# bingjeff/trex-gym

Hardware: AMD Instinct MI355X
Metric: env-steps/sec (whole node), trex.urdf 4096 envs per MI355X (higher is better)
Workload: dtype f32

## Files before the change

trex-gym_amd/csrc/trex_step.hip:

```cpp
#include <hip/hip_runtime.h>
#include <stdint.h>

#include <type_traits>

#include "device_model.h"

#define TL TREX_TL
#define MAXD TREX_MAXD
#define MAXCH TREX_MAXCH
#define MAXC TREX_MAXC

#ifndef TREX_STAMPS
#define TREX_STAMPS 0
#endif
#ifndef TREX_PAIR_MAX
#define TREX_PAIR_MAX 4096
#endif
#ifndef TREX_PAIR_LAUNCH
#define TREX_PAIR_LAUNCH (!TREX_STAMPS)
#endif
#ifndef TREX_ABLATE_EXACT_MATH
#define TREX_ABLATE_EXACT_MATH 0
#endif
#ifndef TREX_ABLATE_EXACT_QUAT
// ... 152 lines not shown
  o[1] = s[1] * v[0] + s[3] * v[1] + s[4] * v[2];
  o[2] = s[2] * v[0] + s[4] * v[1] + s[5] * v[2];
}
__device__ __forceinline__ void sym6_mul(const Sym6 &m, const float *v, float *o) {
  float a[3], b[3], c[3], d[3];
  sym3_mul(m.A, v, a);
  matvec3(m.B, v + 3, b);
  c[0] = m.B[0] * v[0] + m.B[3] * v[1] + m.B[6] * v[2];
  c[1] = m.B[1] * v[0] + m.B[4] * v[1] + m.B[7] * v[2];
  c[2] = m.B[2] * v[0] + m.B[5] * v[1] + m.B[8] * v[2];
  sym3_mul(m.C, v + 3, d);
#pragma unroll
  for (int i = 0; i < 3; i++) { o[i] = a[i] + b[i]; o[3 + i] = c[i] + d[i]; }
}
__device__ __forceinline__ void sym6_full(const Sym6 &m, float *f) {
  const int sidx[3][3] = {{0, 1, 2}, {1, 3, 4}, {2, 4, 5}};
#pragma unroll
  for (int r = 0; r < 3; r++)
#pragma unroll
    for (int c = 0; c < 3; c++) {
      f[6 * r + c] = m.A[sidx[r][c]];
      f[6 * r + 3 + c] = m.B[3 * r + c];
      f[6 * (3 + r) + c] = m.B[3 * c + r];
      f[6 * (3 + r) + 3 + c] = m.C[sidx[r][c]];
    }
}
__device__ __forceinline__ void sym6_rank1_sub(Sym6 &m, const float *U, const float *Us) {
  const int ia[6] = {0, 0, 0, 1, 1, 2}, ib[6] = {0, 1, 2, 1, 2, 2};
#pragma unroll
  for (int k = 0; k < 6; k++) {
    m.A[k] = __builtin_fmaf(-U[ia[k]], Us[ib[k]], m.A[k]);
    m.C[k] = __builtin_fmaf(-U[3 + ia[k]], Us[3 + ib[k]], m.C[k]);
  }
#pragma unroll
  for (int r = 0; r < 3; r++)
#pragma unroll
    for (int c = 0; c < 3; c++) m.B[3 * r + c] = __builtin_fmaf(-U[r], Us[3 + c], m.B[3 * r + c]);
}
__device__ __forceinline__ void cross3_acc(const float *a, const float *b, float &o0, float &o1, float &o2) {
  o0 = __builtin_fmaf(a[1], b[2], __builtin_fmaf(-a[2], b[1], o0));
  o1 = __builtin_fmaf(a[2], b[0], __builtin_fmaf(-a[0], b[2], o1));
  o2 = __builtin_fmaf(a[0], b[1], __builtin_fmaf(-a[1], b[0], o2));
}

struct Chol6 { float l[15], il[6]; };
__device__ __forceinline__ constexpr int lidx(int i, int j) { return i * (i - 1) / 2 + j; }
__device__ __forceinline__ float rsqrt_nr(float s) {
#if TREX_ABLATE_EXACT_MATH
  return 1.0f / sqrtf(s);
#endif
  const float r0 = __builtin_amdgcn_rsqf(s);
  const float e = __builtin_fmaf(-s * r0, r0, 1.0f);
  return __builtin_fmaf(0.5f * r0, e, r0);
}
__device__ __forceinline__ void chol6_factor(const float *a, Chol6 &c) {
#pragma unroll
  for (int j = 0; j < 6; j++) {
    float s = a[6 * j + j];
#pragma unroll
    for (int k = 0; k < j; k++) s -= c.l[lidx(j, k)] * c.l[lidx(j, k)];
    c.il[j] = rsqrt_nr(s);
#pragma unroll
    for (int i = j + 1; i < 6; i++) {
      float t = a[6 * i + j];
#pragma unroll
      for (int k = 0; k < j; k++) t -= c.l[lidx(i, k)] * c.l[lidx(j, k)];
      c.l[lidx(i, j)] = t * c.il[j];
    }
  }
}
__device__ __forceinline__ void chol6_solve(const Chol6 &c, const float *r, float *z) {
  float w[6];
#pragma unroll
  for (int i = 0; i < 6; i++) {
    float t = r[i];
#pragma unroll
    for (int k = 0; k < i; k++) t -= c.l[lidx(i, k)] * w[k];
    w[i] = t * c.il[i];
  }
#pragma unroll
  for (int i = 5; i >= 0; i--) {
    float t = w[i];
#pragma unroll
    for (int k = i + 1; k < 6; k++) t -= c.l[lidx(k, i)] * z[k];
    z[i] = t * c.il[i];
  }
}

constexpr int NJMAX = 25;
constexpr int NROW = NJMAX + 3 * MAXC;
static_assert(NROW == 64, "one constraint row per lane");
#define KROW_LANE(k) ((k) < 3 * MAXC - 1 ? NJMAX + 1 + (k) : 0)
constexpr int CLANE0 = NJMAX + 1;
__device__ __forceinline__ int warm_word(int l) {
  if (l >= 1 && l <= MAXC) return 4 * (l - 1);
  if (l == 0 || l >= CLANE0) { const int k = l == 0 ? 3 * MAXC - 1 : l - CLANE0; return 4 * (k / 3) + 1 + k % 3; }
  return -1;
}
constexpr int BREC = 5;
struct WaveLds {
  float4 body[32 * BREC];
  union {
    struct {
      float aba[32][28];
      float rtab[32][9];
    } t;
    float4 desc[64][4];
    float4 cg[160];
  } u;
  float cpt[MAXC][8];
  float st[6][TL];
  float xch[44];
};
enum { ST_Q, ST_QD, ST_TAU, ST_TARGET, ST_NQD, ST_MDG };
static_assert(sizeof(WaveLds) <= 10240, "16 envs per CU need <= 10 KB of LDS each");
constexpr int CG_WORDS = TREX_CM_WORDS;
struct CgLds {
  unsigned long long best[TL];
  float4 ent[TL][2];
  unsigned cm[CG_WORDS];
};
static_assert(sizeof(CgLds) <= sizeof(WaveLds::u), "contact-generation scratch fits the union area");

struct KernelArgs {
  const TrexDeviceModel *model;
  TrexBatchArrays arr;
  int n_envs;
  const float *actions;
  float *obs;
  float *reward;
  uint8_t *done;
  float *done_f;
  int obs_stride, scal_stride;
  float *penalties;
  const uint8_t *reset_mask;
  int32_t *bal;
  float w_distance, w_energy, w_drift;
  float *debug;
  int n_steps;
  long long step_rows;
  int pen_in_rows;
  float *warm;
  const float *ext;
  float *sens;
};
constexpr int SENS_ROWS = 9;

}

#define WSYNC() do { if (PAIR) __builtin_amdgcn_fence(__ATOMIC_ACQ_REL, "wavefront"); else __syncthreads(); } while (0)
template <bool RESET, bool DEBUG, bool MULTI, bool PAIR = false, bool WARM = false, bool EXT = false, bool SENS = false>
__device__ __forceinline__ void trex_step_body(const KernelArgs &args, const int wg_in) {
  static_assert(!PAIR || (!RESET && !DEBUG && !MULTI), "the pair form exists for the product step launch only");
  static_assert(!(WARM && DEBUG), "the diagnostics dump has no warm-start form");
  static_assert(!EXT || (!RESET && !DEBUG), "the external wrench exists for the product step launches only");
  static_assert(!SENS || !DEBUG, "the diagnostics dump has no contact-sensor form");
  __shared__ WaveLds Wpair[PAIR ? 2 : 1];
  __shared__ __attribute__((aligned(16))) unsigned char Gpair[PAIR ? sizeof(CgLds) : 16];
  const int wave = PAIR ? uni((int)threadIdx.x >> 6) : 0;
  int wave_v = PAIR ? (int)threadIdx.x >> 6 : 0;
  if (PAIR) asm volatile("" : "+v"(wave_v));
  WaveLds &W = Wpair[wave_v];
  __shared__ float4 Wrec[WARM ? (PAIR ? 2 : 1) : 1][MAXC];
  float4 *const Wr = Wrec[WARM ? wave_v : 0];
  const int wg = PAIR ? 2 * wg_in + wave : wg_in;
  const int tid = (int)threadIdx.x & 63;
  const TrexDeviceModel *__restrict__ M = args.model;
  int env = wg;
  int bal_phase = 0;
  if (args.bal) {
    const int32_t *B = args.bal;
    bal_phase = uni(B[TREX_BAL_PHASE]);
    const int32_t *cnt = B + TREX_BAL_COUNTS + TREX_BAL_BINS * bal_phase;
    const int k = wg, q = k >> 10, m = min(1024, args.n_envs - (q << 10));
    int r = q == 0 ? k : (q << 10) + (m - 1 - (k & 1023));
    if (PAIR) {
      const int bq = wg_in >> 9, half = args.n_envs >> 1, bm = min(512, half - (bq << 9));
      const int pidx = bq == 0 ? wg_in : (bq << 9) + (bm - 1 - (wg_in & 511));
      r = wave == 0 ? pidx : args.n_envs - 1 - pidx;
    }
    const int lane_ = tid;
    const int mine = lane_ < TREX_BAL_BINS ? cnt[lane_] : 0;
    int b = TREX_BAL_BINS - 1, total = 0;
#pragma unroll
    for (int c = 0; c < TREX_BAL_BINS; c++) total += rl(mine, c);
    for (; b > 0; b--) {
      const int c = rl(mine, b);
      if (r < c) break;
      r -= c;
    }
    if (total == args.n_envs) {
      env = B[TREX_BAL_LISTS + (size_t)(bal_phase * TREX_BAL_BINS + b) * args.n_envs + r];
      if (env < 0 || env >= args.n_envs) env = wg;
    }
  }
  env = uni(env);

  const int nb = M->nb, maxdepth = M->maxdepth;
  const float dt = PAIR ? uni_sgpr(M->prm[TP_DT]) : M->prm[TP_DT];
  const float inv_dt = PAIR ? uni_sgpr(M->inv_dt) : M->inv_dt;
  const float dt_half = PAIR ? uni_sgpr(0.5f * dt) : 0.5f * dt, dt2_quarter = PAIR ? uni_sgpr(0.25f * dt * dt) : 0.25f * dt * dt;
  const int nj = nb - 1;
  auto Mo = [&]() { const TrexDeviceModel *Mi = M; asm volatile("" : "+s"(Mi)); return Mi; };
  auto lane_id = [&]() {
    int l;
    asm volatile("v_mbcnt_lo_u32_b32 %0, -1, 0\n\tv_mbcnt_hi_u32_b32 %0, -1, %0" : "=v"(l));
    return l;
  };

  float pos[3], quat[4], bv[3], bw[3];
  const float mu = args.arr.domain ? uni(args.arr.friction[env]) : (PAIR ? uni_sgpr(M->prm[TP_FRICTION]) : M->prm[TP_FRICTION]);
  bool motors_on;
  int flags_in = 0, steps_in = 0;
  bool do_reset = false;
  bool bad;
  if (RESET) do_reset = args.reset_mask ? (args.reset_mask[env] != 0) : true;
  if (RESET && !do_reset) {
    if (args.obs && tid >= 1 && tid < nb) {
      float *o = args.obs + (size_t)env * args.obs_stride;
      const int slot = M->obs_slot[tid];
      o[slot] = args.arr.q[(size_t)env * TL + tid];
      o[nj + slot] = args.arr.qd[(size_t)env * TL + tid];
    }
    return;
  }
  {
    const bool is_body = tid < nb, is_joint = tid >= 1 && tid < nb;
    float q = 0.f, qd = 0.f, mtau = 0.f, target = 0.f;
    if (RESET && do_reset) {
#pragma unroll
      for (int c = 0; c < 3; c++) { pos[c] = uni(M->base_pos0[c]); bv[c] = 0.f; bw[c] = 0.f; }
#pragma unroll
      for (int c = 0; c < 4; c++) quat[c] = uni(M->base_quat0[c]);
      q = is_body ? M->q_start[tid & (TL - 1)] : 0.f;
      motors_on = false;
    } else {
      const float *b = args.arr.base + (size_t)env * 16;
#pragma unroll
      for (int c = 0; c < 3; c++) { pos[c] = uni(b[c]); bv[c] = uni(b[7 + c]); bw[c] = uni(b[10 + c]); }
#pragma unroll
      for (int c = 0; c < 4; c++) quat[c] = uni(b[3 + c]);
      flags_in = uni(__float_as_int(b[TREX_BASE_FLAGS]));
      if (tid < TL) {
        q = args.arr.q[(size_t)env * TL + tid];
        qd = args.arr.qd[(size_t)env * TL + tid];
      }
      motors_on = RESET ? ((flags_in & TREX_MOTORS_BIT) != 0) : true;
    }
    steps_in = uni(__float_as_int(args.arr.base[(size_t)env * 16 + TREX_BASE_STEPS]));
    bool badl = !(fabsf(q) < 3.0e38f) || !(fabsf(qd) < 3.0e38f);
#pragma unroll
    for (int k = 0; k < 3; k++) badl |= !(fabsf(pos[k]) < 3.0e38f) || !(fabsf(bv[k]) < 3.0e38f) || !(fabsf(bw[k]) < 3.0e38f);
#pragma unroll
    for (int k = 0; k < 4; k++) badl |= !(fabsf(quat[k]) < 3.0e38f);
    bad = __ballot(badl) != 0ull;
    (void)is_joint;
    if (tid < TL) {
      W.st[ST_Q][tid] = q; W.st[ST_QD][tid] = qd; W.st[ST_TAU][tid] = mtau; W.st[ST_TARGET][tid] = target;
      W.st[ST_NQD][tid] = 0.f;
    }
    if (WARM) {
      const int w = warm_word(tid);
      const float v = RESET ? 0.f : args.warm[(size_t)env * TREX_WARM_WORDS + tid];
      if (w >= 0) reinterpret_cast<float *>(Wr)[w] = v;
    }
  }
  WSYNC();
  const int n_sub = RESET ? (do_reset ? 1 : 0) : M->n_substeps;
#ifndef TREX_PRIO_T1
#define TREX_PRIO_T1 1
#define TREX_PRIO_T2 3
#define TREX_PRIO_T3 6
#endif
  const bool aged_launch = args.n_envs <= 4096;
  const int wave_pair = (wg >> 11) & 1;
  auto set_sweep_priority = [&](int contacts) {
    int v = contacts >= TREX_PRIO_T3 ? 3 : (contacts >= TREX_PRIO_T2 ? 2 : (contacts >= TREX_PRIO_T1 ? 1 : 0));
    v += (aged_launch && wave_pair == 1) ? 1 : 0;
    if (v <= 0) __builtin_amdgcn_s_setprio(0);
    else if (v == 1) __builtin_amdgcn_s_setprio(1);
    else if (v == 2) __builtin_amdgcn_s_setprio(2);
    else __builtin_amdgcn_s_setprio(3);
  };
#ifndef TREX_TREE_HEAVY
#define TREX_TREE_HEAVY 12
#endif
  int prio_nc = 0;
  auto set_tree_priority = [&](int substep) {
    if (!PAIR && TREX_TREE_HEAVY > 0 && prio_nc >= TREX_TREE_HEAVY) { __builtin_amdgcn_s_setprio(3); return; }
    if (aged_launch && ((wave_pair + substep) & 1)) __builtin_amdgcn_s_setprio(1); else __builtin_amdgcn_s_setprio(0);
  };
#if TREX_PRIO_MODE == 1
  if (!RESET) { prio_nc = flags_in & 255; set_tree_priority(0); }
#endif

  const float floor_z = PAIR ? uni_sgpr(M->prm[TP_FLOOR_Z]) : M->prm[TP_FLOOR_Z], margin = PAIR ? uni_sgpr(M->prm[TP_CONTACT_MARGIN]) : M->prm[TP_CONTACT_MARGIN];
  const int iters = M->n_iterations;
  int maxc = M->max_contacts;
  if (maxc > MAXC) maxc = MAXC;

  int stat_nc = 0;
  float stat_imp = 0.f;

  auto forward_kinematics = [&](int lt, int psrc, int depth, float *R, float *r, float *dpar, float *Sa) {
    const TrexDeviceModel *Mi = Mo();
    const int bl = lt & (TL - 1);
    float axis[3], jpos[3], jrot[9];
#pragma unroll
    for (int c = 0; c < 3; c++) { axis[c] = Mi->axis[c][bl]; jpos[c] = Mi->jpos[c][bl]; }
#pragma unroll
    for (int c = 0; c < 9; c++) jrot[c] = Mi->jrot[c][bl];
    const float q = W.st[ST_Q][bl];
    float Rl[9];
    {
      float c = cosf(q), s = sinf(q), t = 1.f - c, rq[9];
      rq[0] = t * axis[0] * axis[0] + c;           rq[1] = t * axis[0] * axis[1] - s * axis[2]; rq[2] = t * axis[0] * axis[2] + s * axis[1];
      rq[3] = t * axis[0] * axis[1] + s * axis[2]; rq[4] = t * axis[1] * axis[1] + c;           rq[5] = t * axis[1] * axis[2] - s * axis[0];
      rq[6] = t * axis[0] * axis[2] - s * axis[1]; rq[7] = t * axis[1] * axis[2] + s * axis[0]; rq[8] = t * axis[2] * axis[2] + c;
      matmul3(jrot, rq, Rl);
    }
    quat_to_mat(quat, R);
    r[0] = r[1] = r[2] = 0.f;
    dpar[0] = dpar[1] = dpar[2] = 0.f;
    for (int d = 1; d <= maxdepth; d++) {
      float pR[9], pr[3];
#pragma unroll
      for (int c = 0; c < 9; c++) pR[c] = wshfl(R[c], psrc);
#pragma unroll
      for (int c = 0; c < 3; c++) pr[c] = wshfl(r[c], psrc);
      if (depth == d) {
        float o[3];
        matmul3(pR, Rl, R);
        matvec3(pR, jpos, o);
#pragma unroll
        for (int c = 0; c < 3; c++) { dpar[c] = o[c]; r[c] = pr[c] + o[c]; }
      }
    }
    matvec3(R, axis, Sa);
    if (!(lt >= 1 && lt < nb)) { Sa[0] = Sa[1] = Sa[2] = 0.f; }
  };

#if TREX_STAMPS
  unsigned long long stamp_last = __builtin_amdgcn_s_memtime();
  int stamp_alive = 0, stamp_lamnz = 0;
  if (args.debug && (threadIdx.x & 63) == 0) args.debug[4096 + 11 * args.n_envs + wg] = (float)env;
#endif
  int age = 0;
  bool time_up = false;
  bool env_bad = false;
  float lift = 0.f, drift = 0.f, energy = 0.f;
  auto finish_step = [&]() {
    const int lt = lane_id();
    const int bl = lt & (TL - 1);
    const bool is_body = lt < nb, is_joint = lt >= 1 && lt < nb;
    float head[3];
    {
      const int parent = is_body ? M->parent[bl] : 0;
      const int psrc = parent < 0 ? 0 : parent;
      const int depth = is_body ? M->depth[bl] : -1;
      float R[9], r[3], dpar[3], Sa[3];
      forward_kinematics(lt, psrc, depth, R, r, dpar, Sa);
      const float hp[3] = {M->head_point[0], M->head_point[1], M->head_point[2]};
      float o[3];
      matvec3(R, hp, o);
      const int hb = M->head_body;
#pragma unroll
      for (int k = 0; k < 3; k++) head[k] = rl(pos[k] + r[k] + o[k], hb);
    }
    float q = W.st[ST_Q][bl], qd = W.st[ST_QD][bl], mtau = W.st[ST_TAU][bl];
    if (lt >= TL) { q = 0.f; qd = 0.f; mtau = 0.f; }
    const float power = wsum(is_joint ? fabsf(qd * mtau) : 0.f);
    lift = uni(args.w_distance * (2.5f - head[2]) * (2.5f - head[2]));
    drift = uni(args.w_drift * (head[0] * head[0] + head[1] * head[1]));
    energy = uni(args.w_energy * power);
    bool badl = !(fabsf(q) < 3.0e38f) || !(fabsf(qd) < 3.0e38f);
#pragma unroll
    for (int k = 0; k < 3; k++) badl |= !(fabsf(pos[k]) < 3.0e38f) || !(fabsf(bv[k]) < 3.0e38f) || !(fabsf(bw[k]) < 3.0e38f);
#pragma unroll
    for (int k = 0; k < 4; k++) badl |= !(fabsf(quat[k]) < 3.0e38f);
    if constexpr (EXT) {
      const float *xw = args.ext + (size_t)env * (6 * TL) + bl;
#pragma unroll
      for (int c = 0; c < 6; c++) badl |= is_body && !(fabsf(xw[c * TL]) < 3.0e38f);
    }
    env_bad = bad || (__ballot(badl) != 0ull);
  };
  auto to_start_pose = [&]() {
#pragma unroll
    for (int k = 0; k < 3; k++) { pos[k] = uni(M->base_pos0[k]); bv[k] = 0.f; bw[k] = 0.f; }
#pragma unroll
    for (int k = 0; k < 4; k++) quat[k] = uni(M->base_quat0[k]);
    const int l = lane_id();
    if (l < TL) {
      W.st[ST_Q][l] = l < nb ? Mo()->q_start[l] : 0.f;
      W.st[ST_QD][l] = 0.f; W.st[ST_TAU][l] = 0.f;
    }
    if (WARM && l < MAXC) Wr[l].x = 0.f;
    WSYNC();
  };
  const int n_launch_steps = MULTI ? args.n_steps : 1;
#pragma unroll 1
  for (int ls = 0; ls < n_launch_steps; ls++) {
  if (!RESET) {
    const int l = lane_id();
    if (l < TL) {
      float target = 0.f;
      if (l >= 1 && l < nb) {
        const TrexDeviceModel *Mi = Mo();
        const float a = args.actions[((size_t)(MULTI ? ls : 0) * args.n_envs + env) * nj + Mi->obs_slot[l]];
        target = fminf(fmaxf(a, Mi->lower[l]), Mi->upper[l]);
      }
      W.st[ST_TARGET][l] = target;
    }
    if (MULTI && ls > 0) { motors_on = true; bad = false; env_bad = false; }
  }
  age = 0; time_up = false;
  if (!RESET && args.arr.max_episode_steps > 0) {
    age = steps_in + 1;
    time_up = age >= args.arr.max_episode_steps;
  }
  const int n_total = n_sub + ((!RESET && time_up) ? 1 : 0);
  int n_loop = n_total;
  int nt_pair[2] = {n_total, n_total};
  if (PAIR) {
    if (lane_id() == 0) W.xch[7] = __int_as_float(n_total);
    __syncthreads();
    nt_pair[0] = uni(__float_as_int(Wpair[0].xch[7])); nt_pair[1] = uni(__float_as_int(Wpair[PAIR ? 1 : 0].xch[7]));
    n_loop = max(nt_pair[0], nt_pair[1]);
  }
#pragma unroll 1
  for (int sub = 0; sub < n_loop; sub++) {
    int lt, bl;
    bool is_body, is_joint;
#define RELANE() do { lt = lane_id(); bl = lt & (TL - 1); is_body = lt < nb; is_joint = lt >= 1 && lt < nb; } while (0)
    int psrc, depth;
    float R[9], r[3];
    float Sa[3], dpar[3];
    int nc = 0;
    const bool act = !PAIR || sub < n_total;
    if (act) {
    if (!RESET && sub == n_sub) {
      finish_step();
      to_start_pose();
      motors_on = false;
    }
    RELANE();
    {
      const TrexDeviceModel *Mi = Mo();
      const int parent = is_body ? Mi->parent[bl] : 0;
      psrc = parent < 0 ? 0 : parent;
      depth = is_body ? Mi->depth[bl] : -1;
    }
    {
      float dpar0[3], Sa0[3];
      forward_kinematics(lt, psrc, depth, R, r, dpar0, Sa0);
      if (lt < TL) {
        float4 *rec = &W.body[BREC * lt];
        rec[0] = make_float4(Sa0[0], Sa0[1], Sa0[2], 0.f);
        rec[1] = make_float4(r[0], r[1], r[2], 0.f);
        rec[3] = make_float4(0.f, 0.f, __int_as_float(psrc + 256 * (depth < 0 ? 255 : depth)), 0.f);
        const TrexDeviceModel *Mi = Mo();
        unsigned ch4 = 0u;
#pragma unroll
        for (int k = 0; k < MAXCH; k++) {
          const int c = is_body ? Mi->child[k][bl] : -1;
          ch4 |= (unsigned)(c < 0 ? 255 : c) << (8 * k);
        }
        rec[4] = make_float4(dpar0[0], dpar0[1], dpar0[2], __uint_as_float(ch4));
      }
    }
    if (PAIR) {
      const int l_ = lane_id();
      if (l_ < TL) {
        float *rt = W.u.t.rtab[l_];
#pragma unroll
        for (int c = 0; c < 9; c++) rt[c] = R[c];
      }
      if (l_ == 0) {
#pragma unroll
        for (int c = 0; c < 3; c++) { W.xch[c] = bw[c]; W.xch[3 + c] = bv[c]; }
        W.xch[6] = __int_as_float(env);
        W.xch[36] = pos[2];
      }
    }
    }
    STAMP(0);
    if (PAIR) { __syncthreads(); SUBSTAMP(16); }
    if (!PAIR || wave == 1) {
    for (int e = 0; e < (PAIR ? 2 : 1); e++) {
    if (PAIR && !(sub < nt_pair[e])) continue;
    WaveLds &E = Wpair[PAIR ? e : 0];
    float posz = pos[2];
    if (PAIR) {
      RELANE();
      posz = E.xch[36];
      if (lt < TL) {
#pragma unroll
        for (int c = 0; c < 9; c++) R[c] = E.u.t.rtab[lt][c];
        const float4 q1_ = E.body[BREC * lt + 1];
        r[0] = q1_.x; r[1] = q1_.y; r[2] = q1_.z;
      }
    }

    nc = 0;
    {
      const TrexDeviceModel *Mi = Mo();
      const int hull_v0 = Mi->hull_start[is_body ? lt : nb], hull_v1 = Mi->hull_start[is_body ? lt + 1 : nb];
      CgLds &G = PAIR ? *reinterpret_cast<CgLds *>(Gpair) : *reinterpret_cast<CgLds *>(&W.u);
      const int nchunk = Mi->nchunk;
      const bool is_chunk = lt < nchunk;
      const int cbody = Mi->chunk_body[bl], cv0 = Mi->chunk_v0[bl], cv1 = is_chunk ? Mi->chunk_v1[bl] : 0;
      float Rz[3], zbc;
      {
        const float zb = posz + r[2] - floor_z;
#pragma unroll
        for (int c = 0; c < 3; c++) Rz[c] = wshfl(R[6 + c], cbody);
        zbc = wshfl(zb, cbody);
      }
      bool near = false;
      if (is_chunk) {
        const float cz = Rz[0] * Mi->chunk_c[0][bl] + Rz[1] * Mi->chunk_c[1][bl] + Rz[2] * Mi->chunk_c[2][bl];
        const float reach = fabsf(Rz[0]) * Mi->chunk_h[0][bl] + fabsf(Rz[1]) * Mi->chunk_h[1][bl] + fabsf(Rz[2]) * Mi->chunk_h[2][bl];
        near = cv1 > cv0 && (zbc + cz - reach < margin);
      }
      const unsigned near_mask = (unsigned)__ballot(near);
      if (near_mask != 0u) {
      {
        unsigned *z = &G.cm[0];
#pragma unroll
        for (int i = 0; i < (CG_WORDS + 63) / 64; i++)
          if (lt + 64 * i < CG_WORDS) z[lt + 64 * i] = 0u;
        if (lt < TL) {
          int ones = -1;
          asm volatile("" : "+v"(ones));
          *reinterpret_cast<int2 *>(&G.best[lt]) = make_int2(ones, ones);
        }
      }
      int total = 0;
      {
        int my_off = 0;
        for (unsigned m = near_mask; m != 0u; m &= m - 1u) {
          const int k = __ffs(m) - 1;
          if (lt == k) my_off = total;
          total += rl(cv1 - cv0, k);
        }
        if (near) {
          const int e = __popc(near_mask & ((1u << bl) - 1u));
          G.ent[e][0] = make_float4(__int_as_float(my_off + (cv1 - cv0)), __int_as_float(cv0 - my_off),
                                    __int_as_float(cbody | (Mi->cm_pack[cbody] << 8)), __int_as_float(Mi->hull_start[cbody]));
          G.ent[e][1] = make_float4(Rz[0], Rz[1], Rz[2], zbc);
        }
      }
      WSYNC();
      SUBSTAMP(9);
      if (total > 0) {
        int cur = 0;
        float4 e0 = G.ent[0][0], e1 = G.ent[0][1];
        constexpr int UN = 4;
        for (int f0 = 0; f0 < total; f0 += 64 * UN) {
          float4 h[UN], q[UN];
          int vtx[UN], rel[UN], bod[UN], mlg[UN], mof[UN];
#pragma unroll
          for (int u = 0; u < UN; u++) {
            const int f = f0 + 64 * u + lt;
            while (f < total && f >= __float_as_int(e0.x)) { cur++; e0 = G.ent[cur][0]; e1 = G.ent[cur][1]; }
            vtx[u] = f < total ? f + __float_as_int(e0.y) : -1;
            bod[u] = __float_as_int(e0.z) & 255;
            mlg[u] = (__float_as_int(e0.z) >> 8) & 255;
            mof[u] = __float_as_int(e0.z) >> 16;
            rel[u] = vtx[u] - __float_as_int(e0.w);
            q[u] = e1;
            h[u] = args.arr.hull[vtx[u] < 0 ? 0 : vtx[u]];
          }
#pragma unroll
          for (int u = 0; u < UN; u++) {
            const float dd = q[u].w + (q[u].x * h[u].x + q[u].y * h[u].y + q[u].z * h[u].z) - h[u].w;
            if (vtx[u] >= 0 && dd < margin) {
              if (mlg[u] != 0 && rel[u] < (32 << mlg[u])) atomicOr(&G.cm[mof[u] + (rel[u] & ((1 << mlg[u]) - 1))], 1u << (rel[u] >> mlg[u]));
              unsigned ub = __float_as_uint(dd);
              ub ^= (ub >> 31) ? 0xffffffffu : 0x80000000u;
              atomicMin(&G.best[bod[u]], ((unsigned long long)ub << 32) | (unsigned)vtx[u]);
            }
          }
        }
      }
      WSYNC();
      SUBSTAMP(10);
      unsigned active_mask = 0u;
      float a_x[3] = {0.f, 0.f, 0.f}, a_d = 0.f;
      int a_v = -1;
      {
        const unsigned long long key = lt < TL ? G.best[bl] : ~0ull;
        if (is_body && key != ~0ull) {
          a_v = (int)(unsigned)(key & 0xffffffffull);
          const float4 hw = args.arr.hull[a_v];
          const float hv[3] = {hw.x, hw.y, hw.z};
          float w[3];
          matvec3(R, hv, w);
          a_x[0] = r[0] + w[0]; a_x[1] = r[1] + w[1]; a_x[2] = r[2] + w[2] - hw.w;
          a_d = posz + a_x[2] - floor_z;
        }
        active_mask = (unsigned)__ballot(a_v >= 0);
      }
      int n_active = __popc(active_mask);
      int K = n_active > 0 ? maxc / n_active : 0;
      K = K > 4 ? 4 : (K < 1 ? 1 : K);
      if (n_active > maxc) {
        int rank = 0;
        for (unsigned m = active_mask; m != 0u; m &= m - 1u) {
          const int b2 = __ffs(m) - 1;
          const float d2 = rl(a_d, b2);
          rank += (d2 < a_d || (d2 == a_d && b2 < lt)) ? 1 : 0;
        }
        active_mask = (unsigned)__ballot(lt < 32 && ((active_mask >> bl) & 1u) && rank < maxc);
        n_active = maxc;
      }
      if (K < 2) {
        const bool mine = lt < 32 && ((active_mask >> bl) & 1u);
        const int slot = __popc(active_mask & ((1u << bl) - 1u));
        if (mine) {
          float *o = E.cpt[slot];
          o[0] = __int_as_float(lt); o[1] = a_x[0]; o[2] = a_x[1]; o[3] = a_x[2]; o[4] = a_d;
          if (WARM) o[5] = __int_as_float(a_v + 1);
        }
        nc = n_active;
      } else {
        const int GS = n_active <= 1 ? 64 : (n_active <= 2 ? 32 : (n_active <= 4 ? 16 : 8));
        const int g = lt & (GS - 1), gi = lt / GS;
        int b = 0;
        bool act = false;
        {
          int i = 0;
          for (unsigned am = active_mask; am != 0u; am &= am - 1u, i++)
            if (gi == i) { b = __ffs(am) - 1; act = true; }
        }
        float Rb[9], rb[3], px[4][3];
        int sel[3] = {-1, -1, -1}, sel3 = -1;
#pragma unroll
        for (int c = 0; c < 9; c++) Rb[c] = wshfl(R[c], b);
#pragma unroll
        for (int c = 0; c < 3; c++) { rb[c] = wshfl(r[c], b); px[0][c] = wshfl(a_x[c], b); }
        sel[0] = act ? wshfl(a_v, b) : -1;
        const int v0 = wshfl(hull_v0, b), v1 = wshfl(hull_v1, b);
        const int cmp = Mi->cm_pack[b & (TL - 1)], mlog = cmp & 255;
        const bool masked = mlog != 0;
        unsigned m0 = 0u, m1 = 0u, m2 = 0u, m3 = 0u;
        if (act && masked) {
          const unsigned *cw = G.cm + (cmp >> 8);
          if (mlog == 3) {
            const unsigned pick = GS >= 64 ? 0x01010101u : (GS >= 32 ? 0x11111111u : (GS >= 16 ? 0x55555555u : 0xFFFFFFFFu));
            m0 = cw[g & 7] & (pick << (g >> 3));
          } else if (GS >= 64) m0 = cw[g & 31] & ((g >> 5) ? 0xAAAAAAAAu : 0x55555555u);
          else if (GS >= 32) m0 = cw[g];
          else if (GS >= 16) { m0 = cw[g]; m1 = cw[g + 16]; }
          else { m0 = cw[g]; m1 = cw[g + 8]; m2 = cw[g + 16]; m3 = cw[g + 24]; }
        }
        const int wstep = (mlog == 3 || GS >= 32) ? 0 : GS;
        const int vmul = mlog == 3 ? 8 : 32, wb0 = mlog == 3 ? (g & 7) : (g & 31);
        int nsel = act ? 1 : 0;
        bool stop = !act;
        constexpr int CC = 4;
        SUBSTAMP(12);
        const bool cached = __ballot(act && (!masked || __popc(m0) + __popc(m1) + __popc(m2) + __popc(m3) > CC)) == 0ull;
        float cx[CC][3];
        int cvx[CC];
#pragma unroll
        for (int u = 0; u < CC; u++) { cvx[u] = -1; cx[u][0] = cx[u][1] = cx[u][2] = 0.f; }
        if (cached) {
          unsigned c0 = m0, c1 = m1, c2 = m2, c3 = m3;
          int wb = wb0;
          float4 hc[CC];
#pragma unroll
          for (int u = 0; u < CC; u++) {
            if (c0 == 0u) { c0 = c1; c1 = c2; c2 = c3; c3 = 0u; wb += wstep; }
            const int j = c0 != 0u ? (__ffs(c0) - 1) : -1;
            c0 &= c0 - 1u;
            cvx[u] = j >= 0 ? v0 + vmul * j + wb : -1;
            hc[u] = args.arr.hull[cvx[u] >= 0 ? cvx[u] : v0];
          }
#pragma unroll
          for (int u = 0; u < CC; u++) {
            const float hv[3] = {hc[u].x, hc[u].y, hc[u].z};
            float w[3];
            matvec3(Rb, hv, w);
            cx[u][0] = rb[0] + w[0]; cx[u][1] = rb[1] + w[1]; cx[u][2] = rb[2] + w[2] - hc[u].w;
            const float dd = posz + cx[u][2] - floor_z;
            if (!(dd < margin)) cvx[u] = -1;
          }
        }
#pragma unroll
        for (int pass = 1; pass < 4; pass++) {
          if (pass >= K || __ballot(!stop) == 0ull) break;
          float bs = -3.0e38f;
          int bi = 0x7fffffff;
          float ex = 0.f, ey = 0.f, flip = 1.f;
          if (pass >= 2) { ex = px[1][0] - px[0][0]; ey = px[1][1] - px[0][1]; }
          if (pass == 3) {
            const float c3 = ex * (px[2][1] - px[0][1]) - ey * (px[2][0] - px[0][0]);
            flip = c3 > 0.f ? -1.f : 1.f;
          }
          float bx[3] = {0.f, 0.f, 0.f};
          auto visit = [&](int v, const float4 h) {
            const float hv[3] = {h.x, h.y, h.z};
            float w[3];
            matvec3(Rb, hv, w);
            const float x0 = rb[0] + w[0], x1 = rb[1] + w[1], x2 = rb[2] + w[2] - h.w;
            const float dd = posz + x2 - floor_z;
            if (!(dd < margin)) return;
            if (v == sel[0] || v == sel[1] || v == sel[2]) return;
            const float dx = x0 - px[0][0], dy = x1 - px[0][1];
            float score;
            if (pass == 1) score = dx * dx + dy * dy;
            else {
              const float cr = ex * dy - ey * dx;
              score = (pass == 2) ? fabsf(cr) : flip * cr;
            }
            if (score > bs || (score == bs && v < bi)) { bs = score; bi = v; bx[0] = x0; bx[1] = x1; bx[2] = x2; }
          };
          if (cached) {
#pragma unroll
            for (int u = 0; u < CC; u++) {
              const int v = cvx[u];
              if (v < 0 || stop || v == sel[0] || v == sel[1] || v == sel[2]) continue;
              const float dx = cx[u][0] - px[0][0], dy = cx[u][1] - px[0][1];
              float score;
              if (pass == 1) score = dx * dx + dy * dy;
              else {
                const float cr = ex * dy - ey * dx;
                score = (pass == 2) ? fabsf(cr) : flip * cr;
              }
              if (score > bs || (score == bs && v < bi)) { bs = score; bi = v; bx[0] = cx[u][0]; bx[1] = cx[u][1]; bx[2] = cx[u][2]; }
            }
          } else if (__ballot(act && !masked) == 0ull) {
            unsigned c0 = stop ? 0u : m0, c1 = stop ? 0u : m1, c2 = stop ? 0u : m2, c3 = stop ? 0u : m3;
            int wb = wb0;
            constexpr int UC = 2;
            while (__ballot((c0 | c1 | c2 | c3) != 0u) != 0ull) {
              int vi[UC];
              float4 hc[UC];
#pragma unroll
              for (int u = 0; u < UC; u++) {
                if (c0 == 0u) { c0 = c1; c1 = c2; c2 = c3; c3 = 0u; wb += wstep; }
                const int j = c0 != 0u ? (__ffs(c0) - 1) : -1;
                c0 &= c0 - 1u;
                vi[u] = j >= 0 ? v0 + vmul * j + wb : -1;
                hc[u] = args.arr.hull[vi[u] >= 0 ? vi[u] : v0];
              }
#pragma unroll
              for (int u = 0; u < UC; u++)
                if (vi[u] >= 0) visit(vi[u], hc[u]);
            }
          } else if (!stop) {
            for (int v = v0 + g; v < v1; v += GS) visit(v, args.arr.hull[v]);
          }
          const int mine = bi;
          const float best = gmaxf(bs, GS);
          bi = gmini(bs == best ? bi : 0x7fffffff, GS);
          if (bi == 0x7fffffff || !(best > 0.f)) stop = true;
          const bool own = !stop && mine == bi;
          {
            const unsigned long long ob = __ballot(own) >> (lt & ~(GS - 1));
            const int src = (lt & ~(GS - 1)) + (ob != 0ull ? __ffsll((unsigned long long)ob) - 1 : 0);
#pragma unroll
            for (int c = 0; c < 3; c++) {
              const float wx = wshfl(bx[c], src);
              if (!stop) px[pass][c] = wx;
            }
          }
          if (!stop) {
            if (pass < 3) sel[pass] = bi;
            else sel3 = bi;
            nsel = pass + 1;
          }
        }
        SUBSTAMP(13);
        int off = 0;
        for (int i = 0; i < n_active; i++) {
          const int ni = rl(nsel, i * GS);
          if (gi > i) off += ni;
          nc += ni;
        }
        if (act && g == 0) {
#pragma unroll
          for (int k = 0; k < 4; k++) {
            if (k < nsel && off + k < maxc) {
// ... 1441 lines not shown
```

Measured before the change: 11.78 million.

## Run paired-env forward kinematics on one wave using both half-wave lane groups

In PAIR mode, forward kinematics for both environments is now computed by wave 0, with lanes 0-31 handling env 0 and lanes 32-63 handling env 1. Before, each wave computed its own env's FK using only its lower TL lanes. Each wave first publishes its base quaternion and state to shared xch, then a barrier, then wave 0 writes the body records and rotation tables for both envs. This uses the otherwise idle upper half-wave lanes and removes duplicated FK work across waves. The cost is an extra __syncthreads per substep and more serialization on wave 0.

```diff
diff --git a/trex-gym_amd/csrc/trex_step.hip b/trex-gym_amd/csrc/trex_step.hip
--- a/trex-gym_amd/csrc/trex_step.hip
+++ b/trex-gym_amd/csrc/trex_step.hip
@@ -478,7 +478,8 @@
   int stat_nc = 0;
   float stat_imp = 0.f;
 
-  auto forward_kinematics = [&](int lt, int psrc, int depth, float *R, float *r, float *dpar, float *Sa) {
+  auto forward_kinematics = [&](const WaveLds &S, int hoff, const float *qb, int lt, int psrc, int depth, float *R, float *r,
+                                float *dpar, float *Sa) {
     const TrexDeviceModel *Mi = Mo();
     const int bl = lt & (TL - 1);
     float axis[3], jpos[3], jrot[9];
@@ -486,7 +487,7 @@
     for (int c = 0; c < 3; c++) { axis[c] = Mi->axis[c][bl]; jpos[c] = Mi->jpos[c][bl]; }
 #pragma unroll
     for (int c = 0; c < 9; c++) jrot[c] = Mi->jrot[c][bl];
-    const float q = W.st[ST_Q][bl];
+    const float q = S.st[ST_Q][bl];
     float Rl[9];
     {
       float c = cosf(q), s = sinf(q), t = 1.f - c, rq[9];
@@ -495,15 +496,15 @@
       rq[6] = t * axis[0] * axis[2] - s * axis[1]; rq[7] = t * axis[1] * axis[2] + s * axis[0]; rq[8] = t * axis[2] * axis[2] + c;
       matmul3(jrot, rq, Rl);
     }
-    quat_to_mat(quat, R);
+    quat_to_mat(qb, R);
     r[0] = r[1] = r[2] = 0.f;
     dpar[0] = dpar[1] = dpar[2] = 0.f;
     for (int d = 1; d <= maxdepth; d++) {
       float pR[9], pr[3];
 #pragma unroll
-      for (int c = 0; c < 9; c++) pR[c] = wshfl(R[c], psrc);
-#pragma unroll
-      for (int c = 0; c < 3; c++) pr[c] = wshfl(r[c], psrc);
+      for (int c = 0; c < 9; c++) pR[c] = wshfl(R[c], psrc + hoff);
+#pragma unroll
+      for (int c = 0; c < 3; c++) pr[c] = wshfl(r[c], psrc + hoff);
       if (depth == d) {
         float o[3];
         matmul3(pR, Rl, R);
@@ -513,7 +514,7 @@
       }
     }
     matvec3(R, axis, Sa);
-    if (!(lt >= 1 && lt < nb)) { Sa[0] = Sa[1] = Sa[2] = 0.f; }
+    if (!(lt - hoff >= 1 && lt - hoff < nb)) { Sa[0] = Sa[1] = Sa[2] = 0.f; }
   };
 
 #if TREX_STAMPS
@@ -535,7 +536,7 @@
       const int psrc = parent < 0 ? 0 : parent;
       const int depth = is_body ? M->depth[bl] : -1;
       float R[9], r[3], dpar[3], Sa[3];
-      forward_kinematics(lt, psrc, depth, R, r, dpar, Sa);
+      forward_kinematics(W, 0, quat, lt, psrc, depth, R, r, dpar, Sa);
       const float hp[3] = {M->head_point[0], M->head_point[1], M->head_point[2]};
       float o[3];
       matvec3(R, hp, o);
@@ -620,18 +621,36 @@
       to_start_pose();
       motors_on = false;
     }
+    }
+    if (PAIR) {
+      if (act && lane_id() == 0) {
+#pragma unroll
+        for (int c = 0; c < 3; c++) { W.xch[c] = bw[c]; W.xch[3 + c] = bv[c]; }
+        W.xch[6] = __int_as_float(env);
+        W.xch[36] = pos[2];
+#pragma unroll
+        for (int c = 0; c < 4; c++) W.xch[37 + c] = quat[c];
+      }
+      __syncthreads(); SUBSTAMP(19);
+    }
+    if (PAIR ? wave == 0 : act) {
     RELANE();
+    const int hoff = PAIR ? (lt & TL) : 0;
+    WaveLds &S = PAIR ? Wpair[lt >> 5] : W;
+    const bool body_l = (PAIR ? bl : lt) < nb;
     {
       const TrexDeviceModel *Mi = Mo();
-      const int parent = is_body ? Mi->parent[bl] : 0;
+      const int parent = body_l ? Mi->parent[bl] : 0;
       psrc = parent < 0 ? 0 : parent;
-      depth = is_body ? Mi->depth[bl] : -1;
+      depth = body_l ? Mi->depth[bl] : -1;
     }
     {
-      float dpar0[3], Sa0[3];
-      forward_kinematics(lt, psrc, depth, R, r, dpar0, Sa0);
-      if (lt < TL) {
-        float4 *rec = &W.body[BREC * lt];
+      float qb[4], dpar0[3], Sa0[3];
+#pragma unroll
+      for (int c = 0; c < 4; c++) qb[c] = PAIR ? S.xch[37 + c] : quat[c];
+      forward_kinematics(S, hoff, qb, lt, psrc, depth, R, r, dpar0, Sa0);
+      if (PAIR ? sub < (hoff ? nt_pair[1] : nt_pair[0]) : lt < TL) {
+        float4 *rec = &S.body[BREC * bl];
         rec[0] = make_float4(Sa0[0], Sa0[1], Sa0[2], 0.f);
         rec[1] = make_float4(r[0], r[1], r[2], 0.f);
         rec[3] = make_float4(0.f, 0.f, __int_as_float(psrc + 256 * (depth < 0 ? 255 : depth)), 0.f);
@@ -639,24 +658,15 @@
         unsigned ch4 = 0u;
 #pragma unroll
         for (int k = 0; k < MAXCH; k++) {
-          const int c = is_body ? Mi->child[k][bl] : -1;
+          const int c = body_l ? Mi->child[k][bl] : -1;
           ch4 |= (unsigned)(c < 0 ? 255 : c) << (8 * k);
         }
         rec[4] = make_float4(dpar0[0], dpar0[1], dpar0[2], __uint_as_float(ch4));
-      }
-    }
-    if (PAIR) {
-      const int l_ = lane_id();
-      if (l_ < TL) {
-        float *rt = W.u.t.rtab[l_];
-#pragma unroll
-        for (int c = 0; c < 9; c++) rt[c] = R[c];
-      }
-      if (l_ == 0) {
-#pragma unroll
-        for (int c = 0; c < 3; c++) { W.xch[c] = bw[c]; W.xch[3 + c] = bv[c]; }
-        W.xch[6] = __int_as_float(env);
-        W.xch[36] = pos[2];
+        if (PAIR) {
+          float *rt = S.u.t.rtab[bl];
+#pragma unroll
+          for (int c = 0; c < 9; c++) rt[c] = R[c];
+        }
       }
     }
     }
```

Result: no change. 11.81 million (median of 6 runs) (+0.3%).
